# PKU-SEC-Lab/FPQVAR

Measured on NVIDIA B200. Metric: fake-quant GB/s over the hot path of one VAR generation pass (config.workload; % of HBM peak = roofline.frac), higher is better.
Workload: dtype f32/f16

## Files before the change

fpqvar_b200/csrc/fpq_rotate.cu:

```cuda
#include "fpq_codes.cuh"
#include "fpq_stream.cuh"

namespace fpq {

struct SignMask { uint32_t w[4]; };

struct Modulate { const float* scale; const float* shift; size_t rows_per_batch; float one; };

struct CodesOut { uint8_t* codes; float* scales; size_t rows_pad; };
constexpr uint32_t CODES_BLOCK_BYTES = 1024;

__device__ __forceinline__ void zero_codes_padding(const CodesOut& co, size_t n_rows, int cpr) {
    const size_t pad = co.rows_pad - n_rows;
    const size_t per_slab = pad * 9;
    const size_t total = per_slab * size_t(cpr);
    for (size_t u = size_t(blockIdx.x) * blockDim.x + threadIdx.x; u < total; u += size_t(gridDim.x) * blockDim.x) {
        const size_t slab = u / per_slab, v = u % per_slab;
        if (v < pad * 8) {
            const size_t row = n_rows + v / 8;
            *reinterpret_cast<uint4*>(co.codes + (slab * (co.rows_pad / 8) + row / 8) * CODES_BLOCK_BYTES + (v & 7) * 128 + (row & 7) * 16) =
                make_uint4(0u, 0u, 0u, 0u);
        } else {
            co.scales[slab * co.rows_pad + n_rows + (v - pad * 8)] = 0.0f;
        }
    }
}

template <class HG>
__device__ __forceinline__ uint4 irregular_codes16(const uint32_t* w, float s, float delta) {
    uint32_t t[8];
#pragma unroll
    for (int i = 0; i < 8; ++i) t[i] = w[i];
    return codes16_h16<HG>(t, s, delta);
}
template <class HG>
static __device__ __noinline__ void codes32_store_h16(const uint32_t* w, float s, float delta, uint8_t* dst) {
    stg_stream(dst, codes16_h16<HG>(w, s, delta));
    stg_stream(dst + 128, codes16_h16<HG>(w + 8, s, delta));
}
template <class HG>
__device__ __forceinline__ void irregular_codes32(const uint32_t* w, float s, float delta, uint8_t* dst) {
    uint32_t t[16];
#pragma unroll
    for (int i = 0; i < 16; ++i) t[i] = w[i];
    codes32_store_h16<HG>(t, s, delta, dst);
}

__device__ __forceinline__ float inv_sqrt128() { return __uint_as_float(0x3DB504F3u); }

__device__ __forceinline__ void load_mult4(const float* __restrict__ smooth, const SignMask& sm, size_t col0, int e0, uint64_t& m01, uint64_t& m23) {
    float4 s4 = make_float4(1.0f, 1.0f, 1.0f, 1.0f);
    if (smooth != nullptr) s4 = __ldg(reinterpret_cast<const float4*>(smooth + col0));
    float f[4] = {s4.x, s4.y, s4.z, s4.w};
    const uint32_t bits = sm.w[e0 >> 5] >> (e0 & 31);
#pragma unroll
    for (int k = 0; k < 4; ++k) {
        f[k] = __fmul_rn(f[k], inv_sqrt128());
        if (!((bits >> k) & 1u)) f[k] = -f[k];
    }
    m01 = pk(f[0], f[1]);
    m23 = pk(f[2], f[3]);
}

__device__ __forceinline__ void load_mod4(const Modulate& mod, size_t off, uint64_t& a01, uint64_t& a23, uint64_t& s01, uint64_t& s23) {
    const float4 sc = __ldg(reinterpret_cast<const float4*>(mod.scale + off));
    const float4 sh = __ldg(reinterpret_cast<const float4*>(mod.shift + off));
    const uint64_t one2 = pk(mod.one, mod.one);
    a01 = fadd2(pk(sc.x, sc.y), one2);
    a23 = fadd2(pk(sc.z, sc.w), one2);
    s01 = pk(sh.x, sh.y);
    s23 = pk(sh.z, sh.w);
}
__device__ __forceinline__ uint64_t modulate2(uint64_t x, uint64_t a, uint64_t sh) {
    const F2 xv = unpk(x), av = unpk(a);
    return fadd2(pk(__fmul_rn(xv.lo, av.lo), __fmul_rn(xv.hi, av.hi)), sh);
}

template <int N>
__device__ __forceinline__ void reg_stage(uint64_t (&P)[N], int h) {
    const uint64_t neg1 = pk(-1.0f, -1.0f);
#pragma unroll
    for (int i = 0; i < N; ++i) {
        if ((i & h) == 0) {
            const uint64_t a = P[i], b = P[i + h];
            P[i] = fadd2(a, b);
            P[i + h] = ffma2(b, neg1, a);
        }
    }
}
template <int N>
__device__ __forceinline__ void pair_stage(uint64_t (&P)[N]) {
#pragma unroll
    for (int i = 0; i < N; ++i) {
        const F2 f = unpk(P[i]);
        P[i] = pk(f.lo + f.hi, f.lo - f.hi);
    }
}

template <int FMT, bool QUANT, bool MOD, bool CODES>
__global__ void __launch_bounds__(256, MOD ? 1 : 0) transform_rotate_quant_small_kernel(const float* __restrict__ x, const float* __restrict__ smooth,
                                                                                       SignMask sm, __half* __restrict__ out, __half* __restrict__ rotated,
                                                                                       size_t n_rows, int cpr, size_t sets_per_col, Modulate mod,
                                                                                       CodesOut co) {
    constexpr int LPG = 8;
    pdl_launch_dependents();
    const int lane = threadIdx.x & 31;
    const int lig = lane % LPG;
    const size_t ls = (size_t(blockIdx.x) * blockDim.x + threadIdx.x) / LPG;
    const int cc = int(ls % size_t(cpr));
    const size_t k0 = ls / size_t(cpr);
    const bool active = k0 < sets_per_col;
    const size_t row_stride = size_t(cpr) * 128;
    const float delta = tie_delta_kernel(uint32_t(ls >> 36));
    const size_t trips = (n_rows + sets_per_col - 1) / sets_per_col;
    pdl_wait();
    uint64_t ms[8];
#pragma unroll
    for (int j = 0; j < 4; ++j) load_mult4(smooth, sm, size_t(cc) * 128 + 32 * j + 4 * lig, 32 * j + 4 * lig, ms[2 * j], ms[2 * j + 1]);
    uint64_t A[MOD ? 8 : 1], SH[MOD ? 8 : 1];
    size_t cur_b = ~size_t(0);
    for (size_t t = 0; t < trips; ++t) {
        const size_t row = MOD ? k0 * trips + t : k0 + t * sets_per_col;
        const bool valid = active && row < n_rows;
        const size_t off = row * row_stride + size_t(cc) * 128;
        uint64_t P[8];
        if (valid) {
#pragma unroll
            for (int j = 0; j < 4; ++j) {
                const uint4 u = ldg_stream(x + off + (j * LPG + lig) * 4);
                P[2 * j] = (uint64_t(u.y) << 32) | u.x;
                P[2 * j + 1] = (uint64_t(u.w) << 32) | u.z;
            }
        } else {
#pragma unroll
            for (int i = 0; i < 8; ++i) P[i] = 0ull;
        }
        if constexpr (MOD) {
            const size_t b = valid ? row / mod.rows_per_batch : cur_b;
            if (b != cur_b) {
                cur_b = b;
                const size_t mo = b * row_stride + size_t(cc) * 128;
#pragma unroll
                for (int j = 0; j < 4; ++j) load_mod4(mod, mo + (j * LPG + lig) * 4, A[2 * j], A[2 * j + 1], SH[2 * j], SH[2 * j + 1]);
            }
#pragma unroll
            for (int i = 0; i < 8; ++i) P[i] = modulate2(P[i], A[i], SH[i]);
        }
#pragma unroll
        for (int i = 0; i < 8; ++i) P[i] = fmul2(P[i], ms[i]);
        pair_stage(P);
        reg_stage(P, 1);
        reg_stage(P, 2);
        reg_stage(P, 4);
#pragma unroll
        for (int o = 1; o < 8; o <<= 1) {
            const float sg = (lig & o) ? -1.0f : 1.0f;
            const uint64_t sg2 = pk(sg, sg);
#pragma unroll
            for (int i = 0; i < 8; ++i) {
                const F2 f = unpk(P[i]);
                const uint64_t q = pk(__shfl_xor_sync(0xffffffffu, f.lo, o), __shfl_xor_sync(0xffffffffu, f.hi, o));
                P[i] = ffma2(P[i], sg2, q);
            }
        }
        uint32_t w[8];
#pragma unroll
        for (int i = 0; i < 8; ++i) w[i] = pack_h2_u64(P[i]);
        if constexpr (CODES) {
            float s;
            const bool ok = sym_quant_tile_h16<FMT, LPG, 8, true, true>(w, s, delta);
            if (valid) {
                const uint4 c = ok ? make_uint4(e4m3x4_h2(w[0], w[1]), e4m3x4_h2(w[2], w[3]), e4m3x4_h2(w[4], w[5]), e4m3x4_h2(w[6], w[7]))
                                   : irregular_codes16<typename SymFmt<FMT>::HG>(w, s, delta);
                uint8_t* cb = co.codes + (size_t(cc) * (co.rows_pad / 8) + row / 8) * CODES_BLOCK_BYTES + (row & 7) * 16 + (lig >> 2) * 128 + (lig & 3) * 4;
                *reinterpret_cast<uint32_t*>(cb) = c.x;
                *reinterpret_cast<uint32_t*>(cb + 256) = c.y;
                *reinterpret_cast<uint32_t*>(cb + 512) = c.z;
                *reinterpret_cast<uint32_t*>(cb + 768) = c.w;
                if (lig == 0) co.scales[size_t(cc) * co.rows_pad + row] = s;
            }
            continue;
        }
        if (valid && rotated != nullptr) {
#pragma unroll
            for (int j = 0; j < 4; ++j) stg_stream(rotated + off + (j * LPG + lig) * 4, make_uint2(w[2 * j], w[2 * j + 1]));
        }
        bool ok = true;
        float s = 0.0f;
        if constexpr (QUANT) ok = sym_quant_tile_h16<FMT, LPG, 8>(w, s, delta);
        if (valid) {
#pragma unroll
            for (int j = 0; j < 4; ++j) stg_stream(out + off + (j * LPG + lig) * 4, make_uint2(w[2 * j], w[2 * j + 1]));
            if (!ok) literal_sym_h16(out + off, out + off, lig, LPG, 4, 4, s, SymFmt<FMT>::GT);
        }
    }
    if constexpr (CODES) zero_codes_padding(co, n_rows, cpr);
}

constexpr bool ROT_HW_QUANT = true;
constexpr int ROT_MIN_CPR = 4, ROT_MAX_CPR = 36;
constexpr int ROT_WARP_STAGE_BYTES = 4096;
constexpr int ROT_WARP_SMEM = 2 * ROT_WARP_STAGE_BYTES + 16;

template <int FMT, bool QUANT, bool MOD, bool CODES>
struct RotStream {
    uint32_t p1;
    uint32_t q1[4];
    uint32_t a2[8];
    bool colok1, colok2;
    int row2;
    int lq;
    uint64_t ms[8];
    uint64_t A[MOD ? 8 : 1], SH[MOD ? 8 : 1];
    float delta;
    const float* pa;
    const float* psh;
    uint32_t left, rpb, row_elems;
    bool reload;
    __half* op;
    __half* rp;
    uint32_t cslab;
    uint32_t crow;

    __device__ __forceinline__ void load_operands() {
        reload = false;
        if (colok1) {
            Modulate m{pa, psh, 0, mod_one};
#pragma unroll
            for (int a = 0; a < 4; ++a) load_mod4(m, size_t(32 * a), A[2 * a], A[2 * a + 1], SH[2 * a], SH[2 * a + 1]);
        }
    }
    __device__ __forceinline__ void pass1(uint32_t buf_off, int nr) {
#pragma unroll
        for (int sub = 0; sub < 2; ++sub) {
            if (sub < nr) {
                if constexpr (MOD) {
                    if (reload) load_operands();
                    if (--left == 0) { left = rpb; pa += row_elems; psh += row_elems; reload = true; }
                }
                {
                    const uint32_t off = buf_off + uint32_t(sub) * 2048u;
                    uint64_t P[8];
#pragma unroll
                    for (int a = 0; a < 4; ++a) {
                        uint4 u;
                        asm volatile("ld.shared.v4.u32 {%0,%1,%2,%3}, [%4];" : "=r"(u.x), "=r"(u.y), "=r"(u.z), "=r"(u.w) : "r"(p1 + off + uint32_t(a * 128)));
                        P[2 * a] = (uint64_t(u.y) << 32) | u.x;
                        P[2 * a + 1] = (uint64_t(u.w) << 32) | u.z;
                    }
                    if constexpr (MOD) {
#pragma unroll
                        for (int i = 0; i < 8; ++i) P[i] = modulate2(P[i], A[i], SH[i]);
                    }
#pragma unroll
                    for (int i = 0; i < 8; ++i) P[i] = fmul2(P[i], ms[i]);
                    pair_stage(P);
                    reg_stage(P, 1);
                    reg_stage(P, 2);
                    reg_stage(P, 4);
                    __syncwarp();
#pragma unroll
                    for (int a = 0; a < 4; ++a) {
                        const F2 p0 = unpk(P[2 * a]), p1v = unpk(P[2 * a + 1]);
                        asm volatile("st.shared.v4.f32 [%0], {%1,%2,%3,%4};" ::"r"(q1[a] + off), "f"(p0.lo), "f"(p0.hi), "f"(p1v.lo), "f"(p1v.hi) : "memory");
                    }
                }
            }
        }
    }
    float mod_one;
    uint32_t lanes8;

    __device__ __forceinline__ void pass2_load(uint32_t buf_off, bool valid, uint64_t (&Q)[16]) {
        (void)valid;
#pragma unroll
        for (int i = 0; i < 8; ++i) {
            uint4 u;
            asm volatile("ld.shared.v4.u32 {%0,%1,%2,%3}, [%4];" : "=r"(u.x), "=r"(u.y), "=r"(u.z), "=r"(u.w) : "r"(a2[i] + buf_off));
            Q[2 * i] = (uint64_t(u.y) << 32) | u.x;
            Q[2 * i + 1] = (uint64_t(u.w) << 32) | u.z;
        }
    }
    __device__ __forceinline__ void pass2_finish(bool valid, uint64_t (&Q)[16], const CodesOut& co) {
        reg_stage(Q, 2);
        reg_stage(Q, 4);
        reg_stage(Q, 8);
        uint32_t w[16];
#pragma unroll
        for (int i = 0; i < 16; ++i) w[i] = pack_h2_u64(Q[i]);
        if constexpr (CODES) {
            float sc;
            const bool ok = sym_quant_tile_h16<FMT, 4, 16, ROT_HW_QUANT, true>(w, sc, delta);
            if (valid) {
                uint8_t* p = co.codes + (size_t(cslab) * (co.rows_pad / 8) + (crow >> 3)) * CODES_BLOCK_BYTES + uint32_t(lq) * 256u + (crow & 7u) * 16u;
                if (ok) {
                    stg_stream(p, make_uint4(e4m3x4_h2(w[0], w[1]), e4m3x4_h2(w[2], w[3]), e4m3x4_h2(w[4], w[5]), e4m3x4_h2(w[6], w[7])));
                    stg_stream(p + 128, make_uint4(e4m3x4_h2(w[8], w[9]), e4m3x4_h2(w[10], w[11]), e4m3x4_h2(w[12], w[13]), e4m3x4_h2(w[14], w[15])));
                } else {
                    irregular_codes32<typename SymFmt<FMT>::HG>(w, sc, delta, p);
                }
                if (lq == 0) co.scales[size_t(cslab) * co.rows_pad + crow] = sc;
            }
            crow += 2;
            return;
        }
        if (rp != nullptr) {
            if (valid) {
#pragma unroll
                for (int q = 0; q < 4; ++q) stg_stream(rp + q * 8, make_uint4(w[4 * q], w[4 * q + 1], w[4 * q + 2], w[4 * q + 3]));
            }
            rp += 2 * size_t(row_elems);
        }
        bool ok = true;
        float sc = 0.0f;
        if constexpr (QUANT) ok = sym_quant_tile_h16<FMT, 4, 16, ROT_HW_QUANT>(w, sc, delta);
        if (valid) {
#pragma unroll
            for (int q = 0; q < 4; ++q) stg_stream(op + q * 8, make_uint4(w[4 * q], w[4 * q + 1], w[4 * q + 2], w[4 * q + 3]));
            if (!ok) literal_sym_h16(op - lq * 32, op - lq * 32, lq, 4, 32, 1, sc, SymFmt<FMT>::GT);
        }
        op += 2 * size_t(row_elems);
    }
};

template <int FMT, bool QUANT, bool MOD, bool CODES>
__device__ __forceinline__ void rotate_stream_body(const float* __restrict__ x, const float* __restrict__ smooth,
                                                   SignMask sm, __half* __restrict__ out, __half* __restrict__ rotated,
                                                   size_t n_rows, int cpr, Modulate mod, const CodesOut& co) {
    extern __shared__ __align__(128) unsigned char smem[];
    const int warp = threadIdx.x >> 5, lane = threadIdx.x & 31;
    const int n_warps = blockDim.x >> 5;
    unsigned char* stage0 = smem + size_t(warp) * (2 * ROT_WARP_STAGE_BYTES);
    uint64_t* full = reinterpret_cast<uint64_t*>(smem + size_t(n_warps) * (2 * ROT_WARP_STAGE_BYTES)) + 2 * warp;
    if (lane == 0) {
        mbar_init(&full[0], 1);
        mbar_init(&full[1], 1);
        mbar_fence_init();
    }
    pdl_launch_dependents();
    __syncwarp();

    const size_t per = n_rows / gridDim.x, rem = n_rows % gridDim.x;
    const size_t r_begin = size_t(blockIdx.x) * per + (blockIdx.x < rem ? blockIdx.x : rem);
    const uint32_t n_mine = uint32_t(per) + (blockIdx.x < rem ? 1u : 0u);
    const uint32_t row_elems = uint32_t(cpr) * 128u;
    const int col0 = 4 * warp;
    const int ncols = cpr - col0 < 4 ? cpr - col0 : 4;

    RotStream<FMT, QUANT, MOD, CODES> st;
    const uint32_t smem_base = smem_u32(stage0);
    const int g4 = lane >> 3, l8 = lane & 7;
    st.colok1 = g4 < ncols;
    st.lanes8 = 0xFFu << (8 * g4);
    st.p1 = smem_base + uint32_t(g4) * 512u + uint32_t(l8) * 16u;
#pragma unroll
    for (int a = 0; a < 4; ++a)
        st.q1[a] = smem_base + uint32_t(g4) * 512u + uint32_t(a) * 128u + ((uint32_t(l8 ^ (g4 & 1)) ^ uint32_t(2 * a)) << 4);
    const int g8 = lane >> 2, c2 = g8 & 3;
    st.lq = lane & 3;
    st.row2 = g8 >> 2;
    st.colok2 = c2 < ncols;
    {
        const uint32_t chunk2 = smem_base + uint32_t(st.row2) * 2048u + uint32_t(c2) * 512u + uint32_t(st.lq) * 128u;
        const uint32_t key2 = uint32_t(2 * st.lq + (g8 & 1));
#pragma unroll
        for (int i = 0; i < 8; ++i) st.a2[i] = chunk2 + ((uint32_t(i) ^ key2) << 4);
    }
    st.delta = tie_delta_kernel(uint32_t((r_begin + size_t(lane)) >> 44));
    st.row_elems = row_elems;
    st.mod_one = mod.one;
    st.op = out + (r_begin + size_t(st.row2)) * row_elems + size_t(col0 + c2) * 128 + st.lq * 32;
    st.rp = rotated != nullptr ? rotated + (r_begin + size_t(st.row2)) * row_elems + size_t(col0 + c2) * 128 + st.lq * 32 : nullptr;
    if constexpr (CODES) {
        st.cslab = uint32_t(col0 + c2);
        st.crow = uint32_t(r_begin) + uint32_t(st.row2);
    }
    st.pa = st.psh = nullptr;
    st.left = st.rpb = 1;
    st.reload = false;
    if constexpr (MOD) {
#pragma unroll
        for (int i = 0; i < 8; ++i) st.A[i] = st.SH[i] = 0ull;
    }
    if constexpr (MOD) {
        const size_t batch = r_begin / mod.rows_per_batch;
        st.rpb = uint32_t(mod.rows_per_batch);
        st.left = st.rpb - uint32_t(r_begin - batch * mod.rows_per_batch);
        const size_t lane_off = batch * row_elems + size_t(col0 + (st.colok1 ? g4 : 0)) * 128 + 4 * l8;
        st.pa = mod.scale + lane_off;
        st.psh = mod.shift + lane_off;
        st.reload = true;
    }
    pdl_wait();

    const unsigned char* gsrc = reinterpret_cast<const unsigned char*>(x + r_begin * row_elems + size_t(col0) * 128);
    const uint32_t row_bytes = uint32_t(ncols) * 512u, row_stride_b = row_elems * 4u;
    uint32_t issued = 0;
    auto issue = [&](uint32_t s) {
        if (issued < n_mine) {
            if (lane == 0) {
                const bool two = n_mine - issued >= 2u;
                mbar_arrive_expect_tx(&full[s], two ? 2u * row_bytes : row_bytes);
                bulk_load(stage0 + s * ROT_WARP_STAGE_BYTES, gsrc, row_bytes, &full[s]);
                if (two) bulk_load(stage0 + s * ROT_WARP_STAGE_BYTES + 2048, gsrc + row_stride_b, row_bytes, &full[s]);
            }
            gsrc += 2 * size_t(row_stride_b);
            issued += 2u;
        }
    };
    issue(0);
    issue(1);
    if constexpr (MOD) st.load_operands();

#pragma unroll
    for (int a = 0; a < 4; ++a) {
        const int e0 = 32 * a + 4 * l8;
        if (st.colok1) load_mult4(smooth, sm, size_t(col0 + g4) * 128 + e0, e0, st.ms[2 * a], st.ms[2 * a + 1]);
        else st.ms[2 * a] = st.ms[2 * a + 1] = 0ull;
    }

    auto step = [&](uint32_t s, uint32_t done, uint32_t phase) {
        const int nr = n_mine - done >= 2u ? 2 : 1;
        const uint32_t buf_off = s * ROT_WARP_STAGE_BYTES;
        mbar_wait(&full[s], phase);
        st.pass1(buf_off, nr);
        __syncwarp();
        const bool valid = st.colok2 && st.row2 < nr;
        uint64_t Q[16];
        st.pass2_load(buf_off, valid, Q);
        asm volatile("fence.proxy.async.shared::cta;" ::: "memory");
        __syncwarp();
        issue(s);
        st.pass2_finish(valid, Q, co);
    };
    uint32_t phase = 0;
    for (uint32_t done = 0; done < n_mine; done += 4u) {
        step(0, done, phase);
        if (done + 2u < n_mine) step(1, done + 2u, phase);
        phase ^= 1u;
    }
    if constexpr (CODES) zero_codes_padding(co, n_rows, cpr);
}

template <int FMT, bool QUANT, bool CODES>
__global__ void __maxnreg__(96) transform_rotate_quant_stream_kernel(const float* __restrict__ x, const float* __restrict__ smooth,
                                                                    SignMask sm, __half* __restrict__ out, __half* __restrict__ rotated,
                                                                    size_t n_rows, int cpr, Modulate mod, CodesOut co) {
    rotate_stream_body<FMT, QUANT, false, CODES>(x, smooth, sm, out, rotated, n_rows, cpr, mod, co);
}
template <int FMT, bool QUANT, bool CODES>
__global__ void __maxnreg__(128) modulate_transform_rotate_quant_stream_kernel(const float* __restrict__ x, const float* __restrict__ smooth,
                                                                              SignMask sm, __half* __restrict__ out, __half* __restrict__ rotated,
                                                                              size_t n_rows, int cpr, Modulate mod, CodesOut co) {
    rotate_stream_body<FMT, QUANT, true, CODES>(x, smooth, sm, out, rotated, n_rows, cpr, mod, co);
}

__global__ void __launch_bounds__(256) transform_rotate_weight_kernel(const float* w, const float* __restrict__ smooth,
                                                                      SignMask sm, float* w_out, size_t n_chunks,
                                                                      int chunks_per_row) {
    const int lane = threadIdx.x & 31;
    const size_t warp_global = (size_t(blockIdx.x) * blockDim.x + threadIdx.x) >> 5;
    const size_t n_warps = (size_t(gridDim.x) * blockDim.x) >> 5;
    for (size_t c = warp_global; c < n_chunks; c += n_warps) {
        const float4 w4 = *reinterpret_cast<const float4*>(w + c * 128 + 4 * lane);
        float f[4] = {w4.x, w4.y, w4.z, w4.w};
        if (smooth != nullptr) {
            const float4 s4 = __ldg(reinterpret_cast<const float4*>(smooth + size_t(c % chunks_per_row) * 128 + 4 * lane));
            f[0] = __fdiv_rn(f[0], s4.x); f[1] = __fdiv_rn(f[1], s4.y);
            f[2] = __fdiv_rn(f[2], s4.z); f[3] = __fdiv_rn(f[3], s4.w);
        }
        double d[4];
#pragma unroll
        for (int k = 0; k < 4; ++k) {
            const int e = 4 * lane + k;
            const bool plus = (sm.w[e >> 5] >> (e & 31)) & 1u;
            d[k] = plus ? double(f[k]) : -double(f[k]);
        }
        { const double a = d[0] + d[1], b = d[0] - d[1], c2 = d[2] + d[3], e2 = d[2] - d[3];
          d[0] = a + c2; d[2] = a - c2; d[1] = b + e2; d[3] = b - e2; }
#pragma unroll
        for (int o = 1; o < 32; o <<= 1) {
            const bool upper = lane & o;
#pragma unroll
            for (int k = 0; k < 4; ++k) {
                const double p = __shfl_xor_sync(0xffffffffu, d[k], o);
                d[k] = upper ? p - d[k] : d[k] + p;
            }
        }
        const double c64 = double(11.313708305358887f);
        float4 o4;
        o4.x = float(d[0] / c64); o4.y = float(d[1] / c64); o4.z = float(d[2] / c64); o4.w = float(d[3] / c64);
        *reinterpret_cast<float4*>(w_out + c * 128 + 4 * lane) = o4;
    }
}

}

using namespace fpq;

struct RotPlan { int warps; int ctas_per_sm; };
static bool rot_plan(int cpr, bool mod, RotPlan& p) {
    if (cpr < ROT_MIN_CPR || cpr > ROT_MAX_CPR) return false;
    p.warps = (cpr + 3) / 4;
    p.ctas_per_sm = (mod ? 16 : 20) / p.warps;
    const int kb = g_tun.smem_kb > 0 ? g_tun.smem_kb : 228;
    const int by_smem = kb * 1024 / (p.warps * ROT_WARP_SMEM + 1024);
    if (p.ctas_per_sm > by_smem) p.ctas_per_sm = by_smem;
    if (p.ctas_per_sm < 1) p.ctas_per_sm = 1;
    return true;
}

template <int FMT, bool QUANT, bool MOD, bool CODES>
static int launch_stream(const float* x, const float* smooth, const SignMask& sm, __half* o, __half* rot, const CodesOut& co, size_t n_rows,
                         int cpr, const RotPlan& plan, const Modulate& m, cudaStream_t st) {
    void (*kernel)(const float*, const float*, SignMask, __half*, __half*, size_t, int, Modulate, CodesOut);
    if constexpr (MOD) kernel = modulate_transform_rotate_quant_stream_kernel<FMT, QUANT, CODES>;
    else kernel = transform_rotate_quant_stream_kernel<FMT, QUANT, CODES>;
    const size_t smem = size_t(plan.warps) * ROT_WARP_SMEM;
    static bool attr_done[64] = {};
    int dev = 0;
    cudaGetDevice(&dev);
    if (!attr_done[dev & 63]) {
        if (cudaFuncSetAttribute(kernel, cudaFuncAttributeMaxDynamicSharedMemorySize, (ROT_MAX_CPR + 3) / 4 * ROT_WARP_SMEM) != cudaSuccess) return FPQ_ERR_CUDA;
        attr_done[dev & 63] = true;
    }
    const size_t steps = (n_rows + 1) / 2;
    const size_t cap = size_t(sm_count()) * plan.ctas_per_sm;
    const unsigned grid = unsigned(steps < cap ? steps : cap);
    launch_pdl(kernel, grid, unsigned(32 * plan.warps), smem, st, x, smooth, sm, o, rot, n_rows, cpr, m, co);
    return finish_launch();
}

template <int FMT, bool QUANT, bool MOD, bool CODES>
static int launch_small(const float* x, const float* smooth, const SignMask& sm, __half* o, __half* rot, const CodesOut& co, size_t n_rows,
                        int cpr, const Modulate& m, cudaStream_t st) {
    const size_t max_sets = size_t(sm_count()) * (MOD ? 1024 : 2048) / 8;
    size_t sets_per_col = max_sets / size_t(cpr);
    if (sets_per_col < 1) sets_per_col = 1;
    if (sets_per_col > n_rows) sets_per_col = n_rows;
    const size_t trips = (n_rows + sets_per_col - 1) / sets_per_col;
    sets_per_col = (n_rows + trips - 1) / trips;
    const size_t n_sets = sets_per_col * size_t(cpr);
    const unsigned grid = unsigned((n_sets + 31) / 32);
    launch_pdl(transform_rotate_quant_small_kernel<FMT, QUANT, MOD, CODES>, grid, 256, 0, st, x, smooth, sm, o, rot, n_rows, cpr, sets_per_col, m, co);
    return finish_launch();
}

template <int FMT, bool QUANT, bool CODES>
static int launch_fmt(const float* x, const Modulate* mod, const float* smooth, const SignMask& sm, __half* o, __half* rot, const CodesOut& co,
                      size_t n_rows, int cpr, cudaStream_t st) {
    const Modulate m = mod ? *mod : Modulate{nullptr, nullptr, 1, 1.0f};
    RotPlan plan;
    const bool big = n_rows * size_t(cpr) > size_t(g_tun.rot_small_max_chunks) && rot_plan(cpr, mod != nullptr, plan) &&
                     (mod == nullptr || mod->rows_per_batch >= 2) &&
                     ((reinterpret_cast<uintptr_t>(o) | reinterpret_cast<uintptr_t>(rot)) & 15) == 0;
    if (big) return mod ? launch_stream<FMT, QUANT, true, CODES>(x, smooth, sm, o, rot, co, n_rows, cpr, plan, m, st)
                        : launch_stream<FMT, QUANT, false, CODES>(x, smooth, sm, o, rot, co, n_rows, cpr, plan, m, st);
    return mod ? launch_small<FMT, QUANT, true, CODES>(x, smooth, sm, o, rot, co, n_rows, cpr, m, st)
               : launch_small<FMT, QUANT, false, CODES>(x, smooth, sm, o, rot, co, n_rows, cpr, m, st);
}

static int check_rotate_args(const float* x, const Modulate* mod, const float* smooth, const uint32_t* sign_bits_host, size_t n_rows, size_t n_cols) {
    if (n_cols == 0 || n_cols % 128 != 0 || n_cols / 128 > 0x7fffffff / 512 || !sign_bits_host || (n_rows && !x)) return FPQ_ERR_ARG;
    if ((reinterpret_cast<uintptr_t>(x) | reinterpret_cast<uintptr_t>(smooth)) & 15) return FPQ_ERR_ARG;
    if (mod != nullptr) {
        if (!mod->scale || !mod->shift || mod->rows_per_batch == 0 || n_rows % mod->rows_per_batch != 0) return FPQ_ERR_ARG;
        if ((reinterpret_cast<uintptr_t>(mod->scale) | reinterpret_cast<uintptr_t>(mod->shift)) & 15) return FPQ_ERR_ARG;
    }
    return FPQ_OK;
}

template <bool CODES>
static int launch_rotate(const float* x, const Modulate* mod, const float* smooth, const uint32_t* sign_bits_host, __half* o, __half* rot,
                         const CodesOut& co, size_t n_rows, size_t n_cols, int format, void* stream) {
    cudaStream_t st = static_cast<cudaStream_t>(stream);
    SignMask sm;
    for (int i = 0; i < 4; ++i) sm.w[i] = sign_bits_host[i];
    const int cpr = int(n_cols / 128);
    switch (format) {
        case FPQ_FMT_E2M1: return launch_fmt<FPQ_FMT_E2M1, true, CODES>(x, mod, smooth, sm, o, rot, co, n_rows, cpr, st);
        case FPQ_FMT_E1M2: return launch_fmt<FPQ_FMT_E1M2, true, CODES>(x, mod, smooth, sm, o, rot, co, n_rows, cpr, st);
        case FPQ_FMT_E3M0: return launch_fmt<FPQ_FMT_E3M0, true, CODES>(x, mod, smooth, sm, o, rot, co, n_rows, cpr, st);
        case FPQ_FMT_E2M3: return launch_fmt<FPQ_FMT_E2M3, true, CODES>(x, mod, smooth, sm, o, rot, co, n_rows, cpr, st);
        case FPQ_FMT_E3M2: return launch_fmt<FPQ_FMT_E3M2, true, CODES>(x, mod, smooth, sm, o, rot, co, n_rows, cpr, st);
        default: break;
    }
    if constexpr (!CODES) return launch_fmt<0, false, false>(x, mod, smooth, sm, o, rot, co, n_rows, cpr, st);
    return FPQ_ERR_ARG;
}

static int launch_rotate_quant(const float* x, const Modulate* mod, const float* smooth, const uint32_t* sign_bits_host, void* out, void* rotated,
                               size_t n_rows, size_t n_cols, int format, void* stream) {
    if (int rc = check_rotate_args(x, mod, smooth, sign_bits_host, n_rows, n_cols)) return rc;
    if ((n_rows && !out) || format < -1 || format >= FPQ_NUM_SYM_FORMATS) return FPQ_ERR_ARG;
    if ((reinterpret_cast<uintptr_t>(out) | reinterpret_cast<uintptr_t>(rotated)) & 7) return FPQ_ERR_ARG;
    if (n_rows == 0) return FPQ_OK;
    return launch_rotate<false>(x, mod, smooth, sign_bits_host, static_cast<__half*>(out), static_cast<__half*>(rotated), CodesOut{nullptr, nullptr, 0},
                                n_rows, n_cols, format, stream);
}

static int launch_rotate_codes(const float* x, const Modulate* mod, const float* smooth, const uint32_t* sign_bits_host, uint8_t* codes, float* scales,
                               size_t n_rows, size_t n_cols, int format, void* stream) {
    if (int rc = check_rotate_args(x, mod, smooth, sign_bits_host, n_rows, n_cols)) return rc;
    if ((n_rows && (!codes || !scales)) || format < 0 || format >= FPQ_NUM_SYM_FORMATS) return FPQ_ERR_ARG;
    if ((reinterpret_cast<uintptr_t>(codes) & 15) || (reinterpret_cast<uintptr_t>(scales) & 3)) return FPQ_ERR_ARG;
    if (n_rows == 0) return FPQ_OK;
    if (fpq_codes_rows_padded(n_rows) > 0xFFFFFFFFull) return FPQ_ERR_UNSUPPORTED;
    return launch_rotate<true>(x, mod, smooth, sign_bits_host, nullptr, nullptr, CodesOut{codes, scales, fpq_codes_rows_padded(n_rows)}, n_rows,
                               n_cols, format, stream);
}

extern "C" int fpq_rotate_plan(int chunks_per_row, int with_modulate, int* plan_host) {
    RotPlan p;
    if (plan_host == nullptr || chunks_per_row < 1) return FPQ_ERR_ARG;
    if (!rot_plan(chunks_per_row, with_modulate != 0, p)) return FPQ_ERR_UNSUPPORTED;
    plan_host[0] = p.warps;
    plan_host[1] = p.ctas_per_sm;
    return FPQ_OK;
}

extern "C" int fpq_transform_rotate_quant(const float* x, const float* smooth, const uint32_t* sign_bits_host, void* out, void* rotated,
                                          size_t n_rows, size_t n_cols, int format, void* stream) {
    return launch_rotate_quant(x, nullptr, smooth, sign_bits_host, out, rotated, n_rows, n_cols, format, stream);
}

extern "C" int fpq_modulate_transform_rotate_quant(const float* x, const float* scale, const float* shift, size_t rows_per_batch,
                                                   const float* smooth, const uint32_t* sign_bits_host, void* out, void* rotated,
                                                   size_t n_rows, size_t n_cols, int format, int flags, void* stream) {
    if (flags & ~FPQ_MOD_GAIN) return FPQ_ERR_ARG;
    const Modulate m{scale, shift, rows_per_batch, (flags & FPQ_MOD_GAIN) ? -0.0f : 1.0f};
    return launch_rotate_quant(x, &m, smooth, sign_bits_host, out, rotated, n_rows, n_cols, format, stream);
}

extern "C" int fpq_transform_rotate_pack_codes(const float* x, const float* smooth, const uint32_t* sign_bits_host, uint8_t* codes, float* scales,
                                               size_t n_rows, size_t n_cols, int format, void* stream) {
    return launch_rotate_codes(x, nullptr, smooth, sign_bits_host, codes, scales, n_rows, n_cols, format, stream);
}

extern "C" int fpq_modulate_transform_rotate_pack_codes(const float* x, const float* scale, const float* shift, size_t rows_per_batch,
                                                        const float* smooth, const uint32_t* sign_bits_host, uint8_t* codes, float* scales,
                                                        size_t n_rows, size_t n_cols, int format, int flags, void* stream) {
    if (flags & ~FPQ_MOD_GAIN) return FPQ_ERR_ARG;
    const Modulate m{scale, shift, rows_per_batch, (flags & FPQ_MOD_GAIN) ? -0.0f : 1.0f};
    return launch_rotate_codes(x, &m, smooth, sign_bits_host, codes, scales, n_rows, n_cols, format, stream);
}

extern "C" int fpq_transform_rotate_weight(const float* w, const float* smooth, const uint32_t* sign_bits_host, float* w_out, size_t n_rows,
                                           size_t n_cols, void* stream) {
    if (n_cols == 0 || n_cols % 128 != 0 || !sign_bits_host || (n_rows && (!w || !w_out))) return FPQ_ERR_ARG;
    if ((reinterpret_cast<uintptr_t>(w) | reinterpret_cast<uintptr_t>(smooth) | reinterpret_cast<uintptr_t>(w_out)) & 15) return FPQ_ERR_ARG;
    if (n_rows == 0) return FPQ_OK;
    cudaStream_t st = static_cast<cudaStream_t>(stream);
    SignMask sm;
    for (int i = 0; i < 4; ++i) sm.w[i] = sign_bits_host[i];
    const int cpr = int(n_cols / 128);
    const size_t n_chunks = n_rows * size_t(cpr);
    transform_rotate_weight_kernel<<<grid_for(n_chunks, 8, 64), 256, 0, st>>>(w, smooth, sm, w_out, n_chunks, cpr);
    return finish_launch();
}
```

Before: 5026.

## Prefetch next row and batch modulation in small rotate kernel, occupancy-sized grid

The small rotate/quant kernel now issues the next row's streaming loads before processing the current row, so load latency overlaps the Hadamard work. It replaces the per-row batch division with a countdown that reloads modulation scale/shift only at batch boundaries, and passes trips as a host-computed argument. Launch bounds for the modulated variant allow two CTAs per SM, and the grid size now comes from a measured occupancy query instead of a fixed constant. The prefetch buffers add registers, which may counteract the higher occupancy target.

```diff
diff --git a/fpqvar_b200/csrc/fpq_rotate.cu b/fpqvar_b200/csrc/fpq_rotate.cu
--- a/fpqvar_b200/csrc/fpq_rotate.cu
+++ b/fpqvar_b200/csrc/fpq_rotate.cu
@@ -97,11 +97,20 @@
     }
 }
 
+__device__ __forceinline__ void load_mod4_raw(const float* scale, const float* shift, uint64_t& a01, uint64_t& a23, uint64_t& s01, uint64_t& s23) {
+    const float4 sc = __ldg(reinterpret_cast<const float4*>(scale));
+    const float4 sh = __ldg(reinterpret_cast<const float4*>(shift));
+    a01 = pk(sc.x, sc.y);
+    a23 = pk(sc.z, sc.w);
+    s01 = pk(sh.x, sh.y);
+    s23 = pk(sh.z, sh.w);
+}
+
 template <int FMT, bool QUANT, bool MOD, bool CODES>
-__global__ void __launch_bounds__(256, MOD ? 1 : 0) transform_rotate_quant_small_kernel(const float* __restrict__ x, const float* __restrict__ smooth,
+__global__ void __launch_bounds__(256, MOD ? 2 : 0) transform_rotate_quant_small_kernel(const float* __restrict__ x, const float* __restrict__ smooth,
                                                                                        SignMask sm, __half* __restrict__ out, __half* __restrict__ rotated,
-                                                                                       size_t n_rows, int cpr, size_t sets_per_col, Modulate mod,
-                                                                                       CodesOut co) {
+                                                                                       size_t n_rows, int cpr, size_t sets_per_col, uint32_t trips,
+                                                                                       Modulate mod, CodesOut co) {
     constexpr int LPG = 8;
     pdl_launch_dependents();
     const int lane = threadIdx.x & 31;
@@ -112,39 +121,64 @@
     const bool active = k0 < sets_per_col;
     const size_t row_stride = size_t(cpr) * 128;
     const float delta = tie_delta_kernel(uint32_t(ls >> 36));
-    const size_t trips = (n_rows + sets_per_col - 1) / sets_per_col;
+    const size_t row0 = MOD ? k0 * trips : k0;
+    const size_t rstep = MOD ? 1 : sets_per_col;
+    const size_t lane_col = size_t(cc) * 128 + size_t(lig) * 4;
+    const size_t rpb = MOD ? mod.rows_per_batch : 1;
+    const size_t b0 = MOD && active ? row0 / rpb : 0;
+    size_t left = MOD ? rpb - (row0 - b0 * rpb) : 0;
+    const float* pa = MOD ? mod.scale + b0 * row_stride + lane_col : nullptr;
+    const float* psh = MOD ? mod.shift + b0 * row_stride + lane_col : nullptr;
     pdl_wait();
+    size_t next_row = row0;
+    bool next_valid = active && next_row < n_rows;
+    uint4 nx[4];
+    const float* xp = x + row0 * row_stride + lane_col;
+    const size_t xstep = rstep * row_stride;
+    auto fetch = [&](bool v) {
+#pragma unroll
+        for (int j = 0; j < 4; ++j) nx[j] = v ? ldg_stream(xp + j * LPG * 4) : make_uint4(0u, 0u, 0u, 0u);
+    };
+    fetch(next_valid);
+    uint64_t A[MOD ? 8 : 1], SH[MOD ? 8 : 1];
+    if constexpr (MOD) {
+#pragma unroll
+        for (int i = 0; i < 8; ++i) A[i] = SH[i] = 0ull;
+        if (next_valid) {
+#pragma unroll
+            for (int j = 0; j < 4; ++j) load_mod4_raw(pa + j * LPG * 4, psh + j * LPG * 4, A[2 * j], A[2 * j + 1], SH[2 * j], SH[2 * j + 1]);
+        }
+    }
     uint64_t ms[8];
 #pragma unroll
     for (int j = 0; j < 4; ++j) load_mult4(smooth, sm, size_t(cc) * 128 + 32 * j + 4 * lig, 32 * j + 4 * lig, ms[2 * j], ms[2 * j + 1]);
-    uint64_t A[MOD ? 8 : 1], SH[MOD ? 8 : 1];
-    size_t cur_b = ~size_t(0);
-    for (size_t t = 0; t < trips; ++t) {
-        const size_t row = MOD ? k0 * trips + t : k0 + t * sets_per_col;
-        const bool valid = active && row < n_rows;
+    for (uint32_t t = 0; t < trips; ++t) {
+        const size_t row = next_row;
+        const bool valid = next_valid;
         const size_t off = row * row_stride + size_t(cc) * 128;
         uint64_t P[8];
-        if (valid) {
-#pragma unroll
-            for (int j = 0; j < 4; ++j) {
-                const uint4 u = ldg_stream(x + off + (j * LPG + lig) * 4);
-                P[2 * j] = (uint64_t(u.y) << 32) | u.x;
-                P[2 * j + 1] = (uint64_t(u.w) << 32) | u.z;
-            }
-        } else {
-#pragma unroll
-            for (int i = 0; i < 8; ++i) P[i] = 0ull;
-        }
+#pragma unroll
+        for (int j = 0; j < 4; ++j) {
+            P[2 * j] = (uint64_t(nx[j].y) << 32) | nx[j].x;
+            P[2 * j + 1] = (uint64_t(nx[j].w) << 32) | nx[j].z;
+        }
+        next_row += rstep;
+        xp += xstep;
+        next_valid = t + 1 < trips && active && next_row < n_rows;
+        fetch(next_valid);
         if constexpr (MOD) {
-            const size_t b = valid ? row / mod.rows_per_batch : cur_b;
-            if (b != cur_b) {
-                cur_b = b;
-                const size_t mo = b * row_stride + size_t(cc) * 128;
-#pragma unroll
-                for (int j = 0; j < 4; ++j) load_mod4(mod, mo + (j * LPG + lig) * 4, A[2 * j], A[2 * j + 1], SH[2 * j], SH[2 * j + 1]);
-            }
-#pragma unroll
-            for (int i = 0; i < 8; ++i) P[i] = modulate2(P[i], A[i], SH[i]);
+            const uint64_t one2 = pk(mod.one, mod.one);
+#pragma unroll
+            for (int i = 0; i < 8; ++i) P[i] = modulate2(P[i], fadd2(A[i], one2), SH[i]);
+            if (--left == 0) {
+                left = rpb;
+                pa += row_stride;
+                psh += row_stride;
+                if (next_valid) {
+#pragma unroll
+                    for (int j = 0; j < 4; ++j) load_mod4_raw(pa + j * LPG * 4, psh + j * LPG * 4, A[2 * j], A[2 * j + 1], SH[2 * j], SH[2 * j + 1]);
+                }
+            }
         }
 #pragma unroll
         for (int i = 0; i < 8; ++i) P[i] = fmul2(P[i], ms[i]);
@@ -534,15 +568,18 @@
 template <int FMT, bool QUANT, bool MOD, bool CODES>
 static int launch_small(const float* x, const float* smooth, const SignMask& sm, __half* o, __half* rot, const CodesOut& co, size_t n_rows,
                         int cpr, const Modulate& m, cudaStream_t st) {
-    const size_t max_sets = size_t(sm_count()) * (MOD ? 1024 : 2048) / 8;
+    const auto kernel = transform_rotate_quant_small_kernel<FMT, QUANT, MOD, CODES>;
+    static int occ[9] = {};
+    const size_t max_sets = size_t(resident_row_grid(kernel, 256, ~size_t(0) >> 8, occ)) * 32;
     size_t sets_per_col = max_sets / size_t(cpr);
     if (sets_per_col < 1) sets_per_col = 1;
     if (sets_per_col > n_rows) sets_per_col = n_rows;
     const size_t trips = (n_rows + sets_per_col - 1) / sets_per_col;
+    if (trips > 0xFFFFFFFFull) return FPQ_ERR_UNSUPPORTED;
     sets_per_col = (n_rows + trips - 1) / trips;
     const size_t n_sets = sets_per_col * size_t(cpr);
     const unsigned grid = unsigned((n_sets + 31) / 32);
-    launch_pdl(transform_rotate_quant_small_kernel<FMT, QUANT, MOD, CODES>, grid, 256, 0, st, x, smooth, sm, o, rot, n_rows, cpr, sets_per_col, m, co);
+    launch_pdl(kernel, grid, 256, 0, st, x, smooth, sm, o, rot, n_rows, cpr, sets_per_col, uint32_t(trips), m, co);
     return finish_launch();
 }
 
```

After: 5089 (median of 6 runs). 1.01x the previous value.
